# colmap/pycolmap

Hardware: AMD Instinct MI355X
Metric: descriptor-pair distances/sec (exhaustive SIFT match: dot + top-2 + ratio + cross-check) (higher is better)
Workload: dtype u8 descriptors, int8 MFMA / int32 accumulate; 1 GPU; 500 images x 4096 descriptors, exhaustive match + ratio test + cross-check (BASELINE.json configs[1] at N=1); pairs_total=124750, pairs_per_rank=124750, kernel=auto, matches_rank0=1865611

## Files before the change

pycolmap_amd/csrc/amc_internal.h:

```cpp
#pragma once

#include <hip/hip_runtime.h>
#include <stdint.h>

#include <algorithm>
#include <cstdlib>
#include <type_traits>
#include <vector>

#include "../../include/amc.h"
#include "guided_region.h"

namespace amc {

constexpr int kDim = AMC_DESC_DIM;
constexpr int kRowPad = 256;
constexpr int kAcosLutSize = 262145;

__host__ __device__ __forceinline__ constexpr uint32_t arena_swizzle(uint32_t row) {
    return ((row >> 1) & 1u) | (((row >> 4) & 3u) << 1);
}

struct ImageDev {
    const uint8_t* raw;
    const uint8_t* prep;
    const int32_t* rs128;
    const float* kp;
    uint32_t rows;
    uint32_t rows_pad;
    uint32_t kp_rows;
    uint32_t pad_;
};

enum : int { kGuidedNone = 0, kGuidedF = 1, kGuidedH = 2 };
struct GuidedDev {
    int32_t kind;
    float max_residual;
    float m[9];
    int32_t grid_ok;
    double bound[2];
    double minv[9];
};

using guided::kGridDim;
struct GridDev {
    const float* sxy;
    const uint32_t* sidx;
    const uint32_t* cell_start;
    float x0, y0, inv_cw, inv_ch;
    float cw, ch;
    float bx1, by1;
    uint32_t n;
    uint32_t pad_;
};
using guided::grid_cell;
#if defined(__HIPCC__)
__device__ __forceinline__ bool guided_rejects(const GuidedDev& g, float x1, float y1, float x2, float y2) {
    const float* m = g.m;
    if (g.kind == kGuidedF) {
        const float Fx1_0 = m[0] * x1 + m[1] * y1 + m[2] * 1.0f;
        const float Fx1_1 = m[3] * x1 + m[4] * y1 + m[5] * 1.0f;
        const float Fx1_2 = m[6] * x1 + m[7] * y1 + m[8] * 1.0f;
        const float Ftx2_0 = m[0] * x2 + m[3] * y2 + m[6] * 1.0f;
        const float Ftx2_1 = m[1] * x2 + m[4] * y2 + m[7] * 1.0f;
        const float x2tFx1 = x2 * Fx1_0 + y2 * Fx1_1 + 1.0f * Fx1_2;
        return x2tFx1 * x2tFx1 / (Fx1_0 * Fx1_0 + Fx1_1 * Fx1_1 + Ftx2_0 * Ftx2_0 + Ftx2_1 * Ftx2_1) > g.max_residual;
    }
    const float Hp_0 = m[0] * x1 + m[1] * y1 + m[2] * 1.0f;
    const float Hp_1 = m[3] * x1 + m[4] * y1 + m[5] * 1.0f;
    const float Hp_2 = m[6] * x1 + m[7] * y1 + m[8] * 1.0f;
    const float e0 = Hp_0 / Hp_2 - x2;
    const float e1 = Hp_1 / Hp_2 - y2;
    return e0 * e0 + e1 * e1 > g.max_residual;
}
#endif

struct Top2 {
    uint32_t best_v;
    uint32_t best_idx;
    uint32_t second_v;
    uint32_t pad;
};

struct PairDev {
    uint32_t slot1, slot2;
    uint32_t mode;
    uint32_t pad;
    uint64_t row_off;
    uint64_t col_off;
};

struct Dot4Work {
    uint32_t pair;
    uint32_t dir;
    uint32_t rb;
};

struct FinalizeParams {
    float max_ratio;
    float max_distance;
    int cross_check;
    int reserved;
};

int api_fail(int code, const char* fmt, ...) __attribute__((format(printf, 2, 3)));

constexpr const char* hipchk_who = nullptr;
#define HIPCHK(expr)                                                                                                   \
    do {                                                                                                               \
        const hipError_t e_ = (expr);                                                                                  \
        if (e_ != hipSuccess)                                                                                          \
            return ::amc::api_fail(AMC_E_HIP, "%s%s%s:%d: %s -> %s", hipchk_who ? hipchk_who : "",                    \
                                   hipchk_who ? ": " : "", __FILE__, __LINE__, #expr, hipGetErrorString(e_));        \
    } while (0)

inline bool env_flag(const char* name) { return std::getenv(name) != nullptr; }
inline long long env_int(const char* name, long long dflt, long long lo, long long hi) {
    const char* e = std::getenv(name);
    return e ? std::min(hi, std::max(lo, std::atoll(e))) : dflt;
}

template <typename T, bool kPinned>
struct GrowBuf {
    T* p = nullptr;
    size_t cap = 0;

    GrowBuf() = default;
    GrowBuf(GrowBuf&& o) noexcept : p(o.p), cap(o.cap) {
        o.p = nullptr;
        o.cap = 0;
    }
    GrowBuf& operator=(GrowBuf&& o) noexcept {
        if (this != &o) {
            release();
            p = o.p;
            cap = o.cap;
            o.p = nullptr;
            o.cap = 0;
        }
        return *this;
    }
    ~GrowBuf() { release(); }

    hipError_t ensure(size_t n) {
        if (n <= cap) return hipSuccess;
        release();
        const size_t want = std::max(n, std::is_void<T>::value ? (size_t)256 : (size_t)16);
        const size_t bytes = want * sizeof(typename std::conditional<std::is_void<T>::value, char, T>::type);
        void* q = nullptr;
        const hipError_t e = kPinned ? hipHostMalloc(&q, bytes, 0) : hipMalloc(&q, bytes);
        if (e == hipSuccess) {
            p = static_cast<T*>(q);
            cap = want;
        }
        return e;
    }
    void release() {
        if (p) (void)(kPinned ? hipHostFree(p) : hipFree(p));
        p = nullptr;
        cap = 0;
    }
};
template <typename T>
using DevBuf = GrowBuf<T, false>;
template <typename T>
using PinBuf = GrowBuf<T, true>;

inline size_t align256(size_t x) { return (x + 255) & ~(size_t)255; }

class DevParts {
  public:
    template <typename T>
    DevParts& part(T** ptr, size_t n) {
        parts_.push_back({ptr, align256(n * sizeof(T)), [](void* q, char* at) { *static_cast<T**>(q) = reinterpret_cast<T*>(at); }});
        return *this;
    }
    hipError_t carve(DevBuf<void>& buf) const {
        size_t total = 0;
        for (const Part& q : parts_) total += q.bytes;
        const hipError_t e = buf.ensure(total);
        if (e != hipSuccess) return e;
        char* at = static_cast<char*>(buf.p);
        for (const Part& q : parts_) {
            q.set(q.ptr, at);
            at += q.bytes;
        }
        return hipSuccess;
    }

  private:
    struct Part {
        void* ptr;
        size_t bytes;
        void (*set)(void* ptr, char* at);
    };
    std::vector<Part> parts_;
};

inline hipError_t create_events(hipEvent_t* ev, int n, const unsigned* flags = nullptr) {
    for (int i = 0; i < n; ++i) {
        const hipError_t e = hipEventCreateWithFlags(&ev[i], flags ? flags[i] : hipEventDefault);
        if (e != hipSuccess) {
            for (int j = 0; j < i; ++j) (void)hipEventDestroy(ev[j]);
            std::fill(ev, ev + n, nullptr);
            return e;
        }
    }
    return hipSuccess;
}

class StreamTimer {
  public:
    explicit StreamTimer(hipStream_t s) : s_(s), made_(create_events(ab_, 2)) {}
    StreamTimer(const StreamTimer&) = delete;
    StreamTimer& operator=(const StreamTimer&) = delete;
    ~StreamTimer() {
        for (hipEvent_t e : ab_)
            if (e) (void)hipEventDestroy(e);
        for (hipEvent_t e : spans_) (void)hipEventDestroy(e);
    }

    hipError_t start() { return made_ != hipSuccess ? made_ : hipEventRecord(ab_[0], s_); }
    hipError_t stop(double& ms) {
        hipError_t e = hipEventRecord(ab_[1], s_);
        if (e == hipSuccess) e = hipEventSynchronize(ab_[1]);
        return e == hipSuccess ? add_elapsed(ab_[0], ab_[1], ms) : e;
    }
    hipError_t span_begin() {
        hipEvent_t two[2];
        if (const hipError_t e = create_events(two, 2)) return e;
        spans_.insert(spans_.end(), two, two + 2);
        return hipEventRecord(two[0], s_);
    }
    hipError_t span_end() { return hipEventRecord(spans_.back(), s_); }
    hipError_t spans(double& ms) const {
        for (size_t i = 0; i + 1 < spans_.size(); i += 2)
            if (const hipError_t e = add_elapsed(spans_[i], spans_[i + 1], ms)) return e;
        return hipSuccess;
    }

  private:
    static hipError_t add_elapsed(hipEvent_t a, hipEvent_t b, double& ms) {
        float f = 0.f;
        const hipError_t e = hipEventElapsedTime(&f, a, b);
        if (e == hipSuccess) ms += f;
        return e;
    }
    hipStream_t s_;
    hipEvent_t ab_[2] = {nullptr, nullptr};
    hipError_t made_;
    std::vector<hipEvent_t> spans_;
};

struct Batches {
    std::vector<size_t> start{0};
    uint64_t most_items = 0, most_elems = 0;
    size_t count() const { return start.size() - 1; }
};
inline Batches split_batches(const uint64_t* offsets, size_t n, uint64_t max_items, uint64_t max_elems,
                             uint64_t factor = 1) {
    Batches b;
    for (size_t i = 0; i < n;) {
        size_t j = i + 1;
        while (j < n && j - i < max_items && (offsets[j + 1] - offsets[i]) * factor <= max_elems) ++j;
        b.most_items = std::max<uint64_t>(b.most_items, j - i);
        b.most_elems = std::max<uint64_t>(b.most_elems, offsets[j] - offsets[i]);
        b.start.push_back(j);
        i = j;
    }
    return b;
}

struct CtxView {
    int device;
    hipStream_t stream;
    const uint32_t* resident;
    uint64_t resident_rows;
};
CtxView ctx_view(amc_ctx* c);
struct TvgPair;
struct VerifyResident {
    size_t npairs = 0;
    uint64_t total = 0;
    const amc_tvg* tvg = nullptr;
    const uint8_t* mask = nullptr;
    const uint64_t* moff = nullptr;
    const TvgPair* tp = nullptr;
    const uint32_t* matches = nullptr;
};
VerifyResident verify_resident(amc_ctx* c);

hipError_t memset_async(void* p, int value, size_t bytes, hipStream_t s);
hipError_t memcpy_async(void* dst, const void* src, size_t bytes, hipMemcpyKind kind, hipStream_t s);

hipError_t launch_prep(const uint8_t* raw, uint8_t* prep, int32_t* rs128, uint32_t rows_pad,
                 uint32_t* maxsq_out, hipStream_t s);

hipError_t launch_match_dot4(const ImageDev* imgs, const PairDev* pairs, const Dot4Work* work,
                       uint32_t nwork, Top2* rowbuf, Top2* colbuf, const GuidedDev* guided, hipStream_t s);
hipError_t launch_match_guided_grid(const ImageDev* imgs, const GridDev* grids, const PairDev* pairs, const Dot4Work* work,
                              uint32_t nwork, Top2* rowbuf, Top2* colbuf, const GuidedDev* guided, hipStream_t s);

constexpr int kSegRows = 128;
constexpr int kSegsPerItem = 8;
struct alignas(64) SegDesc {
    const uint8_t* xprep;
    const int32_t* xrs;
    Top2* out;
    const uint32_t* list;
    const uint8_t* yprep;
    const int32_t* yrs;
    uint32_t cnt;
    uint32_t accword;
    uint32_t yrows;
    uint32_t pad_;
};
__device__ __forceinline__ bool one_way_accepts(const Top2 t, const float* __restrict__ lut,
                                                float max_ratio, float max_distance) {
    if (t.best_v == 0u) return false;
    const float a_best = lut[min(t.best_v, 262144u)];
    if (a_best > max_distance) return false;
    const float a_second = lut[min(t.second_v, 262144u)];
    if (a_best >= max_ratio * a_second) return false;
    return true;
}

hipError_t launch_build_segments(int mode, const ImageDev* imgs, const PairDev* pairs, const uint32_t* order,
                           const uint32_t* grp_start, uint32_t ngroups, const uint32_t* cand_cnt,
                           const uint32_t* candbuf, Top2* outbuf, uint32_t* seg_base, uint32_t* grp_segs,
                           uint32_t* grp_item_base, SegDesc* segs, uint32_t* nitems_dev, hipStream_t s);
struct ScanAccept;
struct CopyJob {
    const void* src = nullptr;
    void* dst = nullptr;
    unsigned long long n16 = 0;
    uint32_t parts = 0, pad_ = 0;
};
hipError_t launch_match_mfma(int mode, const SegDesc* segs, const uint32_t* nitems_dev, uint32_t max_items,
                       uint32_t* queue_head, uint32_t* accmask, const ScanAccept* accept_dev, hipStream_t s,
                       const CopyJob& job = CopyJob(), uint32_t* copy_head = nullptr);

hipError_t launch_resolve_index(int side, const ImageDev* imgs, const PairDev* pairs, uint32_t npairs,
                          Top2* table, uint32_t* accmask, const float* acos_lut, FinalizeParams fp,
                          const uint32_t* cand_cnt, const uint32_t* candbuf, uint32_t* err_count,
                          bool grouped, const uint32_t* order, uint32_t norder, hipStream_t s);
uint32_t resolve_grouped_max_rows();
constexpr uint32_t kSelectMaxCols = 1u << 20;

hipError_t launch_select_candidates(const ImageDev* imgs, const PairDev* pairs, uint32_t npairs, uint32_t max_cols,
                              const Top2* rowbuf, const uint32_t* accmask, const float* acos_lut,
                              FinalizeParams fp, uint32_t* cand_cnt, uint32_t* candbuf, hipStream_t s);

hipError_t launch_finalize(const ImageDev* imgs, const PairDev* pairs, uint32_t npairs,
                     const Top2* rowbuf, const Top2* colbuf, uint32_t* accmask,
                     const float* acos_lut, FinalizeParams fp, uint32_t* cursor, uint32_t capacity,
                     uint32_t* pair_off, uint32_t* pair_cnt, uint32_t* matches, hipStream_t s);

hipError_t launch_host_copy(void* dst_pinned, const void* src_dev, size_t bytes, hipStream_t s);
hipError_t launch_reorder_matches(const uint32_t* src_off, const uint32_t* cnt, const uint64_t* dst_off, uint32_t npairs,
                            const uint32_t* src, uint32_t* dst, hipStream_t s);

struct CameraDev {
    int32_t model_id;
    int32_t has_prior;
    uint64_t width, height;
    double params[12];
};
struct TvgImage {
    const float* kp;
    const double* kp64;
    const double* kpn;
    uint32_t rows;
    uint32_t pad;
    CameraDev cam;
};
hipError_t launch_undistort(const float* kp, const double* kp64, uint32_t rows, const CameraDev& cam, double* kpn,
                            hipStream_t s);
hipError_t launch_project(const double* uv, uint32_t n, const CameraDev& cam, double* xy, hipStream_t s);
struct TvgPair {
    uint32_t slot1, slot2;
    uint64_t match_off;
    uint64_t mask_off;
    uint32_t M;
    uint32_t tab_off[3];
    uint32_t orig;
};
struct PosePair {
    uint32_t slot1, slot2;
    uint64_t match_off;
    uint64_t mask_off;
    uint64_t ws_off;
    uint32_t M;
    int32_t config;
    double E[9], H[9];
};
struct alignas(128) PoseOut {
    int32_t ok;
    int32_t t_is_zero;
    uint32_t num_points3D;
    uint32_t pad;
    double R[9], t[3], q[4], cmed[2];
};
hipError_t launch_pose(const TvgImage* imgs, const PosePair* pairs, uint32_t npairs, const uint32_t* matches,
                       const uint8_t* mask, double* cosine_ws, PoseOut* out, hipStream_t s);

struct alignas(128) TvgOut {
    amc_tvg g;
    unsigned long long prof[8];
    unsigned long long work[12];
};
struct TvgParams {
    int32_t min_num_inliers, detect_watermark, force_H_use, min_num_trials;
    int32_t max_trials[4];
    double min_E_F_inlier_ratio, max_H_inlier_ratio, watermark_min_inlier_ratio,
        watermark_border_size, max_error;
    int32_t force_slow_sampler;
    int32_t no_fast_count;
    int32_t no_fast32;
    int32_t mode;
    uint32_t* bad_index_count;
    const double* wm_cut;
    const uint32_t* stream;
    uint32_t stream_len;
    uint32_t* stream_err;
};
struct alignas(64) TvgEState {
    double model[9];
    double sum;
    int32_t cnt, success, num_trials;
    uint32_t soff;
};
void tvg_diag_report();
void tvg_diag_report_e();
size_t tvg_ws_doubles_host(uint32_t mcap);
size_t tvg_ws_doubles_e_host(uint32_t mcap);
size_t tvg_ws_mask_bytes_host(uint32_t mcap);
constexpr int kTvgEWavesPerSimd = 2;
constexpr int kTvgFhWavesPerSimd = 4;
size_t tvg_lds_bytes(uint32_t mcap, int waves);
size_t tvg_lds_bytes_e(uint32_t mcap, int waves);
hipError_t launch_pack_verify(const TvgOut* out, const TvgPair* tp, uint32_t npairs, const uint8_t* mask_src,
                              const uint64_t* moff, amc_tvg* tvg_dst, uint8_t* mask_dst, unsigned long long* work,
                              int32_t trivial_below, hipStream_t s);
hipError_t launch_homography_decomposition(const double* in27, const double* p1, const double* p2, uint32_t n, double* out16,
                                           double* points3D, hipStream_t s);
hipError_t launch_sampson(const double* p1, const double* p2, size_t n, const double* E9, double* out,
                          hipStream_t s);
hipError_t launch_tvg_e(const TvgImage* imgs, const TvgPair* pairs, uint32_t npairs, const uint32_t* matches,
                        const uint32_t* trial_tabs, const TvgParams& P, double* ws, uint32_t mcap, uint32_t num_waves,
                        int waves_per_block, uint32_t* queue_head, TvgEState* estate, uint8_t* emask, TvgOut* out,
                        uint8_t* out_mask, hipStream_t s);
hipError_t launch_tvg_fh(const TvgImage* imgs, const TvgPair* pairs, uint32_t npairs, const uint32_t* matches,
                         const uint32_t* trial_tabs, const TvgParams& P, double* ws, uint8_t* mask_ws, uint32_t mcap,
                         uint32_t num_waves, int waves_per_block, uint32_t* queue_head, const TvgEState* estate,
                         const uint8_t* emask, TvgOut* out, uint8_t* out_mask, hipStream_t s);

size_t tvg_big_lds_bytes(int waves);
size_t tvg_big_lds_bytes_e(int waves);
size_t tvg_big_idx_doubles_host(uint32_t mcap);
hipError_t launch_tvg_e_big(const TvgImage* imgs, const TvgPair* pairs, uint32_t npairs, const uint32_t* matches,
                            const uint32_t* trial_tabs, const TvgParams& P, double* ws, uint32_t mcap, uint32_t num_waves,
                            int waves_per_block, uint32_t* queue_head, TvgEState* estate, uint8_t* emask, TvgOut* out,
                            uint8_t* out_mask, hipStream_t s);
hipError_t launch_tvg_fh_big(const TvgImage* imgs, const TvgPair* pairs, uint32_t npairs, const uint32_t* matches,
                             const uint32_t* trial_tabs, const TvgParams& P, double* ws, uint8_t* mask_ws, uint32_t mcap,
                             uint32_t num_waves, int waves_per_block, uint32_t* queue_head, const TvgEState* estate,
                             const uint8_t* emask, TvgOut* out, uint8_t* out_mask, hipStream_t s);

}
```

pycolmap_amd/csrc/match_mfma.hip:

```cpp
#include <cstdlib>

#include "amc_internal.h"
#include "scan_accept.h"

namespace amc {

typedef int i32x4 __attribute__((ext_vector_type(4)));
typedef __attribute__((address_space(1))) const void gvoid_t;
typedef __attribute__((address_space(3))) void lvoid_t;

constexpr int kBN = 256;
constexpr int kYS = kBN / 32;
constexpr int kUR = 64;
constexpr int kUPC = kBN / kUR;
constexpr int kChunkBytes = kBN * kDim;
constexpr int kW = kSegsPerItem;
constexpr int kXT = kSegRows / 16;
constexpr int kKeyShift = 7, kKeyCarried = 127;

constexpr int kNB = 3;
constexpr int kOffRs = 0;
constexpr int kOffQ = kOffRs + kNB * kBN * 4;
constexpr int kOffB = kOffQ + 16;
constexpr int kLdsBytes = kOffB + kNB * kChunkBytes;
static_assert(kBN == kRowPad, "a chunk is the row padding unit");
static_assert(kRowPad % kSegRows == 0 && kSegRows % 32 == 0, "segments tile the padded rows");
static_assert(kLdsBytes <= 160 * 1024, "LDS of one CU");
static_assert(sizeof(SegDesc) == 64, "a descriptor is 16 dwords: one per lane of a quarter wave");

enum : int { kDXprep = 0, kDXrs = 2, kDOut = 4, kDList = 6, kDYprep = 8, kDYrs = 10, kDCnt = 12, kDAccword = 13,
             kDYrows = 14 };

__device__ __forceinline__ void mfma_first(i32x4& d, const i32x4& a, const i32x4& b, const i32x4& c) {
    asm volatile("v_mfma_i32_16x16x64_i8 %0, %1, %2, %3" : "=&v"(d) : "v"(a), "v"(b), "v"(c));
}
__device__ __forceinline__ void mfma_acc(i32x4& d, const i32x4& a, const i32x4& b) {
    asm volatile("v_mfma_i32_16x16x64_i8 %0, %1, %2, %0" : "+v"(d) : "v"(a), "v"(b));
}

struct YFrag {
    i32x4 f[2][2];
    i32x4 ci[2];
};

__device__ __noinline__ __attribute__((used)) void copy_part(const uint4* __restrict__ src, uint4* __restrict__ dst,
                                                             unsigned long long b, unsigned long long e, int tid,
                                                             int nthreads) {
    __builtin_assume(tid >= 0 && tid < 1024 && nthreads >= 256 && nthreads <= 512);
    unsigned long long i = b + (unsigned long long)tid;
    const unsigned long long st = (unsigned long long)nthreads;
    for (; i + 3 * st < e; i += 4 * st) {
        const uint4 v0 = src[i], v1 = src[i + st], v2 = src[i + 2 * st], v3 = src[i + 3 * st];
        dst[i] = v0; dst[i + st] = v1; dst[i + 2 * st] = v2; dst[i + 3 * st] = v3;
    }
    for (; i < e; i += st) dst[i] = src[i];
}

template <int MODE>
__global__ __launch_bounds__(64 * kW) void match_mfma_kernel(const SegDesc* __restrict__ segs,
                                                             const uint32_t* __restrict__ nitems_p,
                                                             uint32_t* __restrict__ queue_head,
                                                             uint32_t* __restrict__ accmask,
                                                             const ScanAccept* __restrict__ accept,
                                                             CopyJob job, uint32_t* __restrict__ copy_head) {
    static_assert((kChunkBytes / 1024) % kW == 0 && kYS % (kChunkBytes / 1024 / kW) == 0, "a chunk splits into 1 KiB DMA pieces per wave, dealt evenly over its steps");
    __shared__ __attribute__((aligned(16))) char smem[kLdsBytes];

    const int tid = threadIdx.x;
    const int lane = tid & 63;
    const int wid = __builtin_amdgcn_readfirstlane(tid >> 6);
    const int l15 = lane & 15, lq = lane >> 4;
    volatile uint32_t* s_q = reinterpret_cast<volatile uint32_t*>(smem + kOffQ);
    if constexpr (MODE == 0) {
        if (job.parts) {
            __shared__ uint32_t s_part;
            if (tid == 0) s_part = atomicAdd(copy_head, 1u);
            __syncthreads();
            const uint32_t part = s_part;
            if (part < job.parts)
                copy_part(static_cast<const uint4*>(job.src), static_cast<uint4*>(job.dst), job.n16 * part / job.parts,
                          job.n16 * (part + 1) / job.parts, tid, 64 * kW);
        }
    }
    const uint32_t nitems = *nitems_p;
    const ScanAccept sa = *accept;

    auto load_desc = [&](uint32_t q) -> int {
        int v = 0;
        if (q < nitems && lane < 16) v = reinterpret_cast<const int*>(segs + (size_t)q * kSegsPerItem + wid)[lane];
        return v;
    };
    auto dword = [&](int dv, int f) -> int { return __builtin_amdgcn_readlane(dv, f); };
    auto dptr = [&](int dv, int f) -> const char* {
        const uint64_t lo = (uint32_t)__builtin_amdgcn_readlane(dv, f);
        const uint64_t hi = (uint32_t)__builtin_amdgcn_readlane(dv, f + 1);
        return reinterpret_cast<const char*>(lo | (hi << 32));
    };

    constexpr int kPW = kChunkBytes / 1024 / kW;
    auto stage_piece = [&](const char* yprep, int c, int buf, int ps) __attribute__((always_inline)) {
        const int piece = ps * kW + wid;
        __builtin_amdgcn_global_load_lds((gvoid_t*)(yprep + (size_t)c * kChunkBytes + piece * 1024 + lane * 16),
                                         (lvoid_t*)(smem + kOffB + buf * kChunkBytes + piece * 1024), 16, 0, 0);
    };
    auto stage_rs = [&](const char* yrs, int c, int buf) __attribute__((always_inline)) {
        if (wid == 0)
            __builtin_amdgcn_global_load_lds((gvoid_t*)(yrs + (size_t)c * kBN * 4 + lane * 16),
                                             (lvoid_t*)(smem + kOffRs + buf * kBN * 4), 16, 0, 0);
    };
    auto stage = [&](const char* yprep, const char* yrs, int c, int buf) __attribute__((always_inline)) {
#pragma unroll
        for (int ps = 0; ps < kPW; ++ps) stage_piece(yprep, c, buf, ps);
        stage_rs(yrs, c, buf);
    };

    const int yrow_lane = (kUR / 4) * (l15 >> 2) + (l15 & 3);
    const int ysw_lane = arena_swizzle(yrow_lane);
    const int yoff0 = kOffB + yrow_lane * kDim + ((lq ^ ysw_lane) * 16);
    const int yoff1 = kOffB + yrow_lane * kDim + (((4 + lq) ^ ysw_lane) * 16);
    const int coff = kOffRs + (kUR / 4) * lq * 4;
    auto load_y_part = [&](YFrag& y, int buf, int ys, int part) __attribute__((always_inline)) {
        const int ub = (ys / 2) * kUR, sp = ys % 2;
        if (part < 2) {
            const int so = buf * kBN * 4 + (ub + 8 * sp) * 4;
            y.ci[part] = *reinterpret_cast<const i32x4*>(smem + (coff + so) + 16 * part);
        } else {
            const int tt = (part - 2) >> 1, s = (part - 2) & 1;
            const int so = buf * kChunkBytes + (ub + 8 * sp) * kDim;
            y.f[tt][s] = *reinterpret_cast<const i32x4*>(smem + ((s ? yoff1 : yoff0) + so) + tt * 4 * kDim);
        }
    };
    auto load_y = [&](YFrag& y, int buf, int ys) __attribute__((always_inline)) {
#pragma unroll
        for (int part = 0; part < 6; ++part) load_y_part(y, buf, ys, part);
    };

    i32x4 xf[kXT][2];
    int best[kXT], sec[kXT], btile[kXT], xterm[kXT], part[kXT];
    auto load_x = [&](int dv) __attribute__((always_inline)) {
        const int cnt = dword(dv, kDCnt);
        const char* xprep = dptr(dv, kDXprep);
        const int* xrs = reinterpret_cast<const int*>(dptr(dv, kDXrs));
#pragma unroll
        for (int xt = 0; xt < kXT; ++xt) {
            const int kl = xt * 16 + l15;
            int row;
            if (MODE == 0) {
                row = kl;
            } else {
                const uint32_t* list = reinterpret_cast<const uint32_t*>(dptr(dv, kDList));
                row = cnt > 0 ? (int)list[min(kl, cnt - 1)] : 0;
            }
            const char* rp = xprep + (size_t)row * kDim;
            const int sw = arena_swizzle(row);
#pragma unroll
            for (int s = 0; s < 2; ++s) xf[xt][s] = *reinterpret_cast<const i32x4*>(rp + (((4 * s + lq) ^ sw) * 16));
            xterm[xt] = xrs[row] - (1 << 21);
            best[xt] = ((-xterm[xt]) << kKeyShift) | kKeyCarried;
            sec[xt] = best[xt];
            btile[xt] = -1;
        }
    };

    if (tid == 0) *s_q = atomicAdd(queue_head, 1u);
    __syncthreads();
    uint32_t q = *s_q;
    int dv = load_desc(q);
    if (q < nitems) {
        stage(dptr(dv, kDYprep), dptr(dv, kDYrs), 0, 0);
        if (dword(dv, kDYrows) > kBN) stage(dptr(dv, kDYprep), dptr(dv, kDYrs), 1, 1);
        if (dword(dv, kDCnt) > 0) load_x(dv);
    }
    __syncthreads();

    while (q < nitems) {
        const char* yprep = dptr(dv, kDYprep);
        const char* yrs = dptr(dv, kDYrs);
        const int yrows_item = dword(dv, kDYrows);
        const int nchunks = (yrows_item + kBN - 1) / kBN;
        const int last_steps = (((yrows_item - (nchunks - 1) * kBN) + 31) / 32 + 1) & ~1;
        const bool active = dword(dv, kDCnt) > 0;
        if (tid == 0) *s_q = atomicAdd(queue_head, 1u);

        i32x4 acc[2][2];
        auto insert = [&](int xt, int code) __attribute__((always_inline)) {
            asm volatile(
                "v_lshl_or_b32 %2, %2, 7, %3\n\t"
                "v_med3_i32 %1, %0, %1, %2\n\t"
                "v_max_i32 %0, %0, %2"
                : "+v"(best[xt]), "+v"(sec[xt]), "+v"(part[xt])
                : "s"(code));
        };
        auto flush = [&](int sb) __attribute__((always_inline)) {
#pragma unroll
            for (int xt = 0; xt < kXT; ++xt) {
                const int c = best[xt] & 127;
                btile[xt] = c != kKeyCarried ? sb * 64 + (126 - c) : btile[xt];
                best[xt] |= kKeyCarried;
            }
        };
        auto phase = [&](i32x4 (&an)[2], const YFrag& y, int xtn, const i32x4 (&ac)[2], int xtc, int sp, int gb)
                         __attribute__((always_inline)) {
            mfma_first(an[0], y.f[0][0], xf[xtn][0], y.ci[0]);
            mfma_first(an[1], y.f[1][0], xf[xtn][0], y.ci[1]);
            __builtin_amdgcn_sched_barrier(0);
            if (xtc == 0 ? sp == 0 : sp == 1) {
                insert((xtc + kXT - 1) % kXT, 126 - ((xtc == 0 ? gb - 1 : gb) & 63));
                if (xtc == 0 && gb != 0 && (gb & 63) == 0) flush((gb >> 6) - 1);
                __builtin_amdgcn_sched_barrier(0);
            }
            mfma_acc(an[0], y.f[0][1], xf[xtn][1]);
            mfma_acc(an[1], y.f[1][1], xf[xtn][1]);
            __builtin_amdgcn_sched_barrier(0);
            int t0, t1;
            if (sp == 0)
                asm volatile(
                    "v_max3_i32 %0, %3, %4, %5\n\t"
                    "v_max3_i32 %1, %6, %7, %8\n\t"
                    "v_max3_i32 %0, %0, %9, %10\n\t"
                    "v_max_i32 %2, %0, %1"
                    : "=&v"(t0), "=&v"(t1), "=&v"(part[xtc])
                    : "v"(ac[0][0]), "v"(ac[0][1]), "v"(ac[0][2]), "v"(ac[0][3]), "v"(ac[1][0]), "v"(ac[1][1]),
                      "v"(ac[1][2]), "v"(ac[1][3]));
            else
                asm volatile(
                    "v_max3_i32 %0, %3, %4, %5\n\t"
                    "v_max3_i32 %1, %6, %7, %8\n\t"
                    "v_max3_i32 %0, %0, %9, %10\n\t"
                    "v_max3_i32 %2, %0, %1, %2"
                    : "=&v"(t0), "=&v"(t1), "+v"(part[xtc])
                    : "v"(ac[0][0]), "v"(ac[0][1]), "v"(ac[0][2]), "v"(ac[0][3]), "v"(ac[1][0]), "v"(ac[1][1]),
                      "v"(ac[1][2]), "v"(ac[1][3]));
            __builtin_amdgcn_sched_barrier(0);
        };

        YFrag y0, y1;
        asm volatile("s_waitcnt vmcnt(0)" ::: "memory");
        __syncthreads();
        const uint32_t qn = *s_q;
        const int dvn = load_desc(qn);
        if (active) {
            load_y(y0, 0, 0);
            mfma_first(acc[0][0], y0.f[0][0], xf[0][0], y0.ci[0]);
            mfma_first(acc[0][1], y0.f[1][0], xf[0][0], y0.ci[1]);
            mfma_acc(acc[0][0], y0.f[0][1], xf[0][1]);
            mfma_acc(acc[0][1], y0.f[1][1], xf[0][1]);
            part[kXT - 1] = -(1 << 24);
            __builtin_amdgcn_sched_barrier(0);
        }
        auto step = [&](YFrag& yc, YFrag& yn, int c, int cb, int nb, int ys, int sp) __attribute__((always_inline)) {
            const bool lastt = (ys == kYS - 1);
            const bool cross = lastt && (c + 1 < nchunks);
            const bool fetch = c + 2 < nchunks;
            if (fetch) {
                const int fb = cb == 0 ? 2 : cb - 1;
                constexpr int kEvery = kYS / kPW;
                static_assert(kEvery == 2, "a DMA piece per block, behind its first step");
                if (sp == 0) stage_piece(yprep, c + 2, fb, ys / kEvery);
                if (ys == 0) stage_rs(yrs, c + 2, fb);
            }
            if (cross) {
                if (!fetch) asm volatile("s_waitcnt vmcnt(0)" ::: "memory");
                else if (wid == 0) asm volatile("s_waitcnt vmcnt(%0)" ::"n"(kPW + 1) : "memory");
                else asm volatile("s_waitcnt vmcnt(%0)" ::"n"(kPW) : "memory");
                asm volatile("s_barrier" ::: "memory");
            }
            if (active) {
                const int nbuf = cross ? nb : cb;
                const int nys = lastt ? (cross ? 0 : ys) : ys + 1;
                const int gb = c * kUPC + ys / 2;
#pragma unroll
                for (int xt = 0; xt < kXT; ++xt) {
                    if (xt + 1 < kXT)
                        phase(acc[(xt + 1) & 1], yc, xt + 1, acc[xt & 1], xt, sp, gb);
                    else
                        phase(acc[0], yn, 0, acc[xt & 1], xt, sp, gb);
                    if (xt < 6) {
                        load_y_part(yn, nbuf, nys, xt);
                        __builtin_amdgcn_sched_barrier(0);
                    }
                }
            }
        };
        for (int c = 0, cb = 0; c < nchunks; ++c) {
            const int nb = cb == 2 ? 0 : cb + 1;
            const int yend = (c == nchunks - 1) ? last_steps : kYS;
#pragma unroll 1
            for (int ys = 0; ys < yend; ys += 2) {
                step(y0, y1, c, cb, nb, ys, 0);
                step(y1, y0, c, cb, nb, ys + 1, 1);
            }
            cb = nb;
        }
        if (active) {
            const int lastb = (nchunks - 1) * kUPC + last_steps / 2 - 1;
            insert(kXT - 1, 126 - (lastb & 63));
            flush(lastb >> 6);
#pragma unroll
            for (int xt = 0; xt < kXT; ++xt) {
                best[xt] >>= kKeyShift;
                sec[xt] >>= kKeyShift;
            }
        }
        __syncthreads();

        int eb[kXT], es[kXT], et[kXT], ex[kXT];
#pragma unroll
        for (int xt = 0; xt < kXT; ++xt) {
            asm volatile("v_mov_b32 %0, %1" : "=v"(eb[xt]) : "v"(best[xt]));
            asm volatile("v_mov_b32 %0, %1" : "=v"(es[xt]) : "v"(sec[xt]));
            asm volatile("v_mov_b32 %0, %1" : "=v"(et[xt]) : "v"(btile[xt]));
            ex[xt] = xterm[xt];
        }
        if (qn < nitems) {
            stage(dptr(dvn, kDYprep), dptr(dvn, kDYrs), 0, 0);
            if (dword(dvn, kDYrows) > kBN) stage(dptr(dvn, kDYprep), dptr(dvn, kDYrs), 1, 1);
            if (dword(dvn, kDCnt) > 0) load_x(dvn);
        }
        if (active) {
            const int cnt = dword(dv, kDCnt);
            uint32_t bits_lo = 0;
#pragma unroll
            for (int xt = 0; xt < kXT; ++xt) {
                const int kl = xt * 16 + l15;
                int b = eb[xt], s = es[xt], t = et[xt] < 0 ? -1 : et[xt] * 2 + (lq >> 1);
#pragma unroll
                for (int m = 16; m <= 32; m <<= 1) {
                    const int ob = __shfl_xor(b, m);
                    const int os = __shfl_xor(s, m);
                    const int ot = __shfl_xor(t, m);
                    const bool ow = (ob > b) || (ob == b && (unsigned)ot < (unsigned)t);
                    s = max(max(s, os), ow ? b : ob);
                    t = ow ? ot : t;
                    b = ow ? ob : b;
                }
                bool acc_bit = false;
                if (lq == 0 && kl < cnt) {
                    Top2* out = reinterpret_cast<Top2*>(const_cast<char*>(dptr(dv, kDOut)));
                    int row = kl;
                    if (MODE == 1) row = (int)reinterpret_cast<const uint32_t*>(dptr(dv, kDList))[kl];
                    Top2 o;
                    o.best_v = (uint32_t)(b + ex[xt]);
                    o.best_idx = o.best_v ? (uint32_t)t : 0xFFFFFFFFu;
                    o.second_v = (uint32_t)(s + ex[xt]);
                    o.pad = 0;
                    out[row] = o;
                    if (MODE == 0) acc_bit = scan_may_accept(sa, o.best_v, o.second_v);
                }
                if (MODE == 0) {
                    const uint32_t bits = (uint32_t)__ballot(acc_bit);
                    if (xt & 1) {
                        if (lane == 0) accmask[(uint32_t)dword(dv, kDAccword) + (xt >> 1)] = bits_lo | (bits << 16);
                    } else {
                        bits_lo = bits;
                    }
                }
            }
        }
        q = qn;
        dv = dvn;
    }
}

__device__ __forceinline__ uint32_t pair_segments(int mode, const ImageDev* imgs, const PairDev& p, uint32_t pi,
                                                  const uint32_t* cand_cnt, uint32_t* nrows_out) {
    const uint32_t nx = mode == 0 ? imgs[p.slot1].rows : cand_cnt[pi];
    const uint32_t ny = imgs[mode == 0 ? p.slot2 : p.slot1].rows;
    *nrows_out = nx;
    return ny ? (nx + kSegRows - 1) / kSegRows : 0u;
}

__global__ __launch_bounds__(256) void seg_count_kernel(int mode, const ImageDev* __restrict__ imgs,
                                                        const PairDev* __restrict__ pairs,
                                                        const uint32_t* __restrict__ order,
                                                        const uint32_t* __restrict__ grp_start,
                                                        const uint32_t* __restrict__ cand_cnt,
                                                        uint32_t* __restrict__ seg_base, uint32_t* __restrict__ grp_segs) {
    __shared__ uint32_t wsum[4];
    const uint32_t g = blockIdx.x, tid = threadIdx.x, lane = tid & 63, wid = tid >> 6;
    const uint32_t i0 = grp_start[g], i1 = grp_start[g + 1];
    uint32_t running = 0;
    for (uint32_t base = i0; base < i1; base += 256) {
        const uint32_t i = base + tid;
        uint32_t s = 0, nr;
        if (i < i1) {
            const uint32_t pi = order[i];
            s = pair_segments(mode, imgs, pairs[pi], pi, cand_cnt, &nr);
        }
        uint32_t inc = s;
#pragma unroll
        for (int m = 1; m < 64; m <<= 1) {
            const uint32_t o = __shfl_up(inc, m);
            if (lane >= (uint32_t)m) inc += o;
        }
        if (lane == 63) wsum[wid] = inc;
        __syncthreads();
        uint32_t wbase = 0, total = 0;
        for (uint32_t k = 0; k < 4; ++k) {
            if (k < wid) wbase += wsum[k];
            total += wsum[k];
        }
        if (i < i1) seg_base[i] = running + wbase + inc - s;
        running += total;
        __syncthreads();
    }
    if (tid == 0) grp_segs[g] = running;
}

__global__ __launch_bounds__(1024) void seg_scan_kernel(const uint32_t* __restrict__ grp_segs, uint32_t ngroups,
                                                        uint32_t* __restrict__ grp_item_base,
                                                        uint32_t* __restrict__ nitems_out) {
    __shared__ uint32_t wsum[16];
    const uint32_t tid = threadIdx.x, lane = tid & 63, wid = tid >> 6;
    uint32_t running = 0;
    for (uint32_t base = 0; base < ngroups; base += 1024) {
        const uint32_t g = base + tid;
        const uint32_t s = g < ngroups ? (grp_segs[g] + kSegsPerItem - 1) / kSegsPerItem : 0u;
        uint32_t inc = s;
#pragma unroll
        for (int m = 1; m < 64; m <<= 1) {
            const uint32_t o = __shfl_up(inc, m);
            if (lane >= (uint32_t)m) inc += o;
        }
        if (lane == 63) wsum[wid] = inc;
        __syncthreads();
        uint32_t wbase = 0, total = 0;
        for (uint32_t k = 0; k < 16; ++k) {
            if (k < wid) wbase += wsum[k];
            total += wsum[k];
        }
        if (g < ngroups) grp_item_base[g] = running + wbase + inc - s;
        running += total;
        __syncthreads();
    }
    if (tid == 0) *nitems_out = running;
}

constexpr uint32_t kFillY = 8;
__global__ __launch_bounds__(256) void seg_fill_kernel(int mode, const ImageDev* __restrict__ imgs,
                                                       const PairDev* __restrict__ pairs,
                                                       const uint32_t* __restrict__ order,
                                                       const uint32_t* __restrict__ grp_start,
                                                       const uint32_t* __restrict__ cand_cnt,
                                                       const uint32_t* __restrict__ candbuf,
                                                       const uint32_t* __restrict__ seg_base,
                                                       const uint32_t* __restrict__ grp_segs,
                                                       const uint32_t* __restrict__ grp_item_base,
                                                       Top2* __restrict__ outbuf, SegDesc* __restrict__ segs) {
    const uint32_t g = blockIdx.x, tid = threadIdx.x, lane = tid & 63, wid = blockIdx.y * 4 + (tid >> 6);
    const uint32_t i0 = grp_start[g], i1 = grp_start[g + 1];
    if (i0 >= i1) return;
    const uint32_t total = grp_segs[g];
    if (total == 0) return;
    SegDesc* gs = segs + (size_t)grp_item_base[g] * kSegsPerItem;
    const PairDev p0 = pairs[order[i0]];
    const ImageDev Y = imgs[mode == 0 ? p0.slot2 : p0.slot1];
    for (uint32_t i = i0 + wid; i < i1; i += 4 * kFillY) {
        const uint32_t pi = order[i];
        const PairDev p = pairs[pi];
        uint32_t nx;
        const uint32_t ns = pair_segments(mode, imgs, p, pi, cand_cnt, &nx);
        const ImageDev X = imgs[mode == 0 ? p.slot1 : p.slot2];
        const uint32_t sb = seg_base[i];
        for (uint32_t k = lane; k < ns; k += 64) {
            const uint32_t row0 = k * kSegRows;
            SegDesc d;
            d.yprep = Y.prep;
            d.yrs = Y.rs128;
            d.yrows = Y.rows;
            d.cnt = min(nx - row0, (uint32_t)kSegRows);
            d.pad_ = 0;
            if (mode == 0) {
                d.xprep = X.prep + (size_t)row0 * kDim;
                d.xrs = X.rs128 + row0;
                d.out = outbuf + p.row_off + row0;
                d.list = nullptr;
                d.accword = (uint32_t)((p.row_off + row0) >> 5);
            } else {
                d.xprep = X.prep;
                d.xrs = X.rs128;
                d.out = outbuf + p.col_off;
                d.list = candbuf + p.col_off + row0;
                d.accword = 0;
            }
            gs[sb + k] = d;
        }
    }
    const uint32_t padded = (total + kSegsPerItem - 1) / kSegsPerItem * kSegsPerItem;
    if (blockIdx.y == 0 && tid < padded - total) {
        SegDesc d;
        d.xprep = Y.prep;
        d.xrs = Y.rs128;
        d.out = nullptr;
        d.list = nullptr;
        d.yprep = Y.prep;
        d.yrs = Y.rs128;
        d.cnt = 0;
        d.accword = 0;
        d.yrows = Y.rows;
        d.pad_ = 0;
        gs[total + tid] = d;
    }
}

hipError_t launch_build_segments(int mode, const ImageDev* imgs, const PairDev* pairs, const uint32_t* order,
                                 const uint32_t* grp_start, uint32_t ngroups, const uint32_t* cand_cnt,
                                 const uint32_t* candbuf, Top2* outbuf, uint32_t* seg_base, uint32_t* grp_segs,
                                 uint32_t* grp_item_base, SegDesc* segs, uint32_t* nitems_dev, hipStream_t s) {
    if (ngroups == 0) return memset_async(nitems_dev, 0, sizeof(uint32_t), s);
    hipLaunchKernelGGL(seg_count_kernel, dim3(ngroups), dim3(256), 0, s, mode, imgs, pairs, order, grp_start,
                       cand_cnt, seg_base, grp_segs);
    hipLaunchKernelGGL(seg_scan_kernel, dim3(1), dim3(1024), 0, s, grp_segs, ngroups, grp_item_base, nitems_dev);
    hipLaunchKernelGGL(seg_fill_kernel, dim3(ngroups, kFillY), dim3(256), 0, s, mode, imgs, pairs, order, grp_start,
                       cand_cnt, candbuf, seg_base, grp_segs, grp_item_base, outbuf, segs);
    return hipGetLastError();
}

hipError_t launch_match_mfma(int mode, const SegDesc* segs, const uint32_t* nitems_dev, uint32_t max_items,
                             uint32_t* queue_head, uint32_t* accmask, const ScanAccept* accept_dev, hipStream_t s,
                             const CopyJob& job_in, uint32_t* copy_head) {
    if (max_items == 0) return hipSuccess;
    CopyJob job = (mode == 0 && copy_head) ? job_in : CopyJob();
    hipError_t e = job.parts ? memset_async(copy_head, 0, sizeof(uint32_t), s) : hipSuccess;
    if (e != hipSuccess) return e;
    int dev = 0, cus = 256;
    if ((e = hipGetDevice(&dev)) != hipSuccess) return e;
    if ((e = hipDeviceGetAttribute(&cus, hipDeviceAttributeMultiprocessorCount, dev)) != hipSuccess) return e;
    static const int grid_cap = [] {
        const char* e = std::getenv("AMC_SCAN_GRID");
        return e ? std::atoi(e) : 0;
    }();
    if (grid_cap > 0 && grid_cap < cus) cus = grid_cap;
    const uint32_t grid = max_items < (uint32_t)cus ? max_items : (uint32_t)cus;
    if (job.parts > grid) job.parts = grid;
    if ((e = memset_async(queue_head, 0, sizeof(uint32_t), s)) != hipSuccess) return e;
    if (mode == 0)
        hipLaunchKernelGGL((match_mfma_kernel<0>), dim3(grid), dim3(64 * kW), 0, s, segs, nitems_dev, queue_head,
                           accmask, accept_dev, job, copy_head);
    else
        hipLaunchKernelGGL((match_mfma_kernel<1>), dim3(grid), dim3(64 * kW), 0, s, segs, nitems_dev, queue_head,
                           accmask, accept_dev, job, copy_head);
    return hipGetLastError();
}

}
```

Measured before the change: 12780 billion distances/s.

## Widen the MFMA scan unit to 128 rows with four steps per loop block

Doubles the row block (kUR 64→128) so each lane quarter covers a 32-row tile. The Y scan loop is unrolled to four steps per block, with the tile index math, last-step rounding and DMA piece cadence adjusted to match. The arena swizzle is shifted to row bits 5-6 so the LDS bank spread fits the new row mapping. The aim is to halve top-2 insert/flush overhead per row and to cut loop and branch cost, at the price of more unrolled code and register pressure. Optional timestamp instrumentation behind AMC_SCAN_STAMPS and an A/B summary script are added.

```diff
diff --git a/profiles/scan128/recipes/ab_summary.py b/profiles/scan128/recipes/ab_summary.py
--- /dev/null
+++ b/profiles/scan128/recipes/ab_summary.py
@@ -0,0 +1,57 @@
+import json, sys, os, statistics
+d, out = sys.argv[1], sys.argv[2]
+def last_json(p):
+    if not os.path.exists(p): return None
+    for line in reversed(open(p).read().strip().split("\n")):
+        line = line.strip()
+        if line.startswith("{"):
+            try: return json.loads(line)
+            except Exception: pass
+    return None
+def leg_ms(j, leg):
+    if leg in ("headline", "headline_of_the_full_runs"): return j.get("ms_per_step")
+    if leg == "scan_ms_per_launch": return (j.get("roofline") or {}).get("avg_kernel_ms")
+    v = j.get(leg)
+    if not isinstance(v, dict): return None
+    for k in ("ms_per_step", "ms_per_call", "ms"):
+        if k in v: return v[k]
+    return None
+res = {
+    "cmd": ["python bench.py --gpus 1 --steps 20 --warmup 5", "python bench.py --full --no-db --no-config3 --no-config4"],
+    "how": "one GPU call (profiles/scan128/recipes/ab_parent.sh), alternating parent1 / new1 / parent2 / new2 / parent3 / new3; parent = the parent commit's library (tools/ab_prev_lib.sh) selected with AMC_LIB_PATH, new = the tree's own library; each step under its own timeout, chained with &&.  The db leg is left out: it goes through the host module, which links libamc.so directly and cannot be switched this way.",
+    "rule": "headline: the new median must be below the parent's median by more than three times the parent's max - min of this call (gain_over_three_spreads).  Every other leg: the new median may exceed the parent's median by at most the parent's max - min (within_parent_spread).",
+    "ms_per_step": {}, "summary": {}, "other": {}}
+runs = {}
+for kind in ("head", "full"):
+    for who in ("parent", "new"):
+        for i in (1, 2, 3):
+            runs[(kind, who, i)] = last_json(f"{d}/{kind}_{who}{i}.json")
+legs = [("headline", "head"), ("scan_ms_per_launch", "head")]
+legs += [(l, "full") for l in ("headline_of_the_full_runs", "verify", "pipeline", "dense", "ragged", "sift_stats")]
+for leg, kind in legs:
+    vals = {}
+    for who in ("parent", "new"):
+        for i in (1, 2, 3):
+            j = runs[(kind, who, i)]
+            if j is not None:
+                v = leg_ms(j, leg)
+                if v is not None: vals[f"{who}{i}"] = round(float(v), 3)
+    res["ms_per_step"][leg] = vals
+    p = [vals[k] for k in vals if k.startswith("parent")]
+    n = [vals[k] for k in vals if k.startswith("new")]
+    if len(p) == 3 and len(n) == 3:
+        pm, nm, sp = statistics.median(p), statistics.median(n), max(p) - min(p)
+        res["summary"][leg] = {"parent_median": pm, "new_median": nm, "parent_spread": round(sp, 3),
+                               "new_minus_parent": round(nm - pm, 3), "within_parent_spread": nm - pm <= sp,
+                               "gain_over_three_spreads": pm - nm > 3 * sp}
+for (kind, who, i), j in runs.items():
+    if j is None or kind != "full": continue
+    o = {}
+    for leg in ("ragged", "sift_stats", "dense", "pipeline", "verify", "cpu_baseline"):
+        v = j.get(leg)
+        if isinstance(v, dict):
+            o[leg] = {k: v[k] for k in ("vs_uniform", "gpu_vs_oracle_mismatching_pairs", "value") if k in v}
+    res["other"][f"{who}{i}"] = o
+json.dump(res, open(out, "w"), indent=1)
+print(json.dumps(res["summary"], indent=1))
+print(json.dumps(res["other"]))
diff --git a/pycolmap_amd/csrc/amc_internal.h b/pycolmap_amd/csrc/amc_internal.h
--- a/pycolmap_amd/csrc/amc_internal.h
+++ b/pycolmap_amd/csrc/amc_internal.h
@@ -18,7 +18,7 @@
 constexpr int kAcosLutSize = 262145;
 
 __host__ __device__ __forceinline__ constexpr uint32_t arena_swizzle(uint32_t row) {
-    return ((row >> 1) & 1u) | (((row >> 4) & 3u) << 1);
+    return ((row >> 1) & 1u) | (((row >> 5) & 3u) << 1);
 }
 
 struct ImageDev {
diff --git a/pycolmap_amd/csrc/match_mfma.hip b/pycolmap_amd/csrc/match_mfma.hip
--- a/pycolmap_amd/csrc/match_mfma.hip
+++ b/pycolmap_amd/csrc/match_mfma.hip
@@ -11,7 +11,8 @@
 
 constexpr int kBN = 256;
 constexpr int kYS = kBN / 32;
-constexpr int kUR = 64;
+constexpr int kUR = 128;
+constexpr int kSPB = kUR / 32;
 constexpr int kUPC = kBN / kUR;
 constexpr int kChunkBytes = kBN * kDim;
 constexpr int kW = kSegsPerItem;
@@ -24,6 +25,7 @@
 constexpr int kOffB = kOffQ + 16;
 constexpr int kLdsBytes = kOffB + kNB * kChunkBytes;
 static_assert(kBN == kRowPad, "a chunk is the row padding unit");
+static_assert(kUR == 128 && kSPB == 4, "a lane quarter's rows of a block are one 32-row tile; the loop body is one block");
 static_assert(kRowPad % kSegRows == 0 && kSegRows % 32 == 0, "segments tile the padded rows");
 static_assert(kLdsBytes <= 160 * 1024, "LDS of one CU");
 static_assert(sizeof(SegDesc) == 64, "a descriptor is 16 dwords: one per lane of a quarter wave");
@@ -42,6 +44,12 @@
     i32x4 f[2][2];
     i32x4 ci[2];
 };
+
+#ifdef AMC_SCAN_STAMPS
+constexpr int kStampMaxWG = 1024;
+__device__ uint32_t g_scan_stamps[2 * kStampMaxWG * kSegsPerItem * 8];
+#define AMC_STAMP() ((uint32_t)__builtin_amdgcn_s_memtime())
+#endif
 
 __device__ __noinline__ __attribute__((used)) void copy_part(const uint4* __restrict__ src, uint4* __restrict__ dst,
                                                              unsigned long long b, unsigned long long e, int tid,
@@ -120,7 +128,7 @@
     const int yoff1 = kOffB + yrow_lane * kDim + (((4 + lq) ^ ysw_lane) * 16);
     const int coff = kOffRs + (kUR / 4) * lq * 4;
     auto load_y_part = [&](YFrag& y, int buf, int ys, int part) __attribute__((always_inline)) {
-        const int ub = (ys / 2) * kUR, sp = ys % 2;
+        const int ub = (ys / kSPB) * kUR, sp = ys % kSPB;
         if (part < 2) {
             const int so = buf * kBN * 4 + (ub + 8 * sp) * 4;
             y.ci[part] = *reinterpret_cast<const i32x4*>(smem + (coff + so) + 16 * part);
@@ -162,6 +170,11 @@
         }
     };
 
+#ifdef AMC_SCAN_STAMPS
+    uint32_t st_a = 0, st_first = 0, st_end = 0, st_sum[5] = {0, 0, 0, 0, 0};
+    bool st_prev = false, st_prev_active = false;
+    uint32_t* const st_slot = g_scan_stamps + ((size_t)(MODE * kStampMaxWG + min((int)blockIdx.x, kStampMaxWG - 1)) * kW + wid) * 8;
+#endif
     if (tid == 0) *s_q = atomicAdd(queue_head, 1u);
     __syncthreads();
     uint32_t q = *s_q;
@@ -178,7 +191,7 @@
         const char* yrs = dptr(dv, kDYrs);
         const int yrows_item = dword(dv, kDYrows);
         const int nchunks = (yrows_item + kBN - 1) / kBN;
-        const int last_steps = (((yrows_item - (nchunks - 1) * kBN) + 31) / 32 + 1) & ~1;
+        const int last_steps = (((yrows_item - (nchunks - 1) * kBN) + 31) / 32 + kSPB - 1) & ~(kSPB - 1);
         const bool active = dword(dv, kDCnt) > 0;
         if (tid == 0) *s_q = atomicAdd(queue_head, 1u);
 
@@ -204,7 +217,7 @@
             mfma_first(an[0], y.f[0][0], xf[xtn][0], y.ci[0]);
             mfma_first(an[1], y.f[1][0], xf[xtn][0], y.ci[1]);
             __builtin_amdgcn_sched_barrier(0);
-            if (xtc == 0 ? sp == 0 : sp == 1) {
+            if (xtc == 0 ? sp == 0 : sp == kSPB - 1) {
                 insert((xtc + kXT - 1) % kXT, 126 - ((xtc == 0 ? gb - 1 : gb) & 63));
                 if (xtc == 0 && gb != 0 && (gb & 63) == 0) flush((gb >> 6) - 1);
                 __builtin_amdgcn_sched_barrier(0);
@@ -239,6 +252,24 @@
         __syncthreads();
         const uint32_t qn = *s_q;
         const int dvn = load_desc(qn);
+#ifdef AMC_SCAN_STAMPS
+        {
+            const uint32_t now = AMC_STAMP();
+            if (st_prev) {
+                st_sum[0] += st_a;
+                st_sum[1] += now - st_end;
+                st_sum[2] += now - st_first;
+                st_sum[3] += 1;
+                st_sum[4] += st_prev_active ? 1 : 0;
+                if (lane == 0) {
+#pragma unroll
+                    for (int k = 0; k < 5; ++k) st_slot[k] = st_sum[k];
+                }
+            }
+            st_a = 0;
+            st_first = now;
+        }
+#endif
         if (active) {
             load_y(y0, 0, 0);
             mfma_first(acc[0][0], y0.f[0][0], xf[0][0], y0.ci[0]);
@@ -249,26 +280,32 @@
             __builtin_amdgcn_sched_barrier(0);
         }
         auto step = [&](YFrag& yc, YFrag& yn, int c, int cb, int nb, int ys, int sp) __attribute__((always_inline)) {
-            const bool lastt = (ys == kYS - 1);
+            const bool lastt = sp == kSPB - 1 && ys == kYS - 1;
             const bool cross = lastt && (c + 1 < nchunks);
             const bool fetch = c + 2 < nchunks;
             if (fetch) {
                 const int fb = cb == 0 ? 2 : cb - 1;
                 constexpr int kEvery = kYS / kPW;
-                static_assert(kEvery == 2, "a DMA piece per block, behind its first step");
-                if (sp == 0) stage_piece(yprep, c + 2, fb, ys / kEvery);
+                static_assert(kEvery == 2, "a DMA piece behind every other step");
+                if (sp % kEvery == 0) stage_piece(yprep, c + 2, fb, ys / kEvery);
                 if (ys == 0) stage_rs(yrs, c + 2, fb);
             }
             if (cross) {
+#ifdef AMC_SCAN_STAMPS
+                const uint32_t st_t = AMC_STAMP();
+#endif
                 if (!fetch) asm volatile("s_waitcnt vmcnt(0)" ::: "memory");
                 else if (wid == 0) asm volatile("s_waitcnt vmcnt(%0)" ::"n"(kPW + 1) : "memory");
                 else asm volatile("s_waitcnt vmcnt(%0)" ::"n"(kPW) : "memory");
                 asm volatile("s_barrier" ::: "memory");
+#ifdef AMC_SCAN_STAMPS
+                st_a += AMC_STAMP() - st_t;
+#endif
             }
             if (active) {
                 const int nbuf = cross ? nb : cb;
                 const int nys = lastt ? (cross ? 0 : ys) : ys + 1;
-                const int gb = c * kUPC + ys / 2;
+                const int gb = c * kUPC + ys / kSPB;
 #pragma unroll
                 for (int xt = 0; xt < kXT; ++xt) {
                     if (xt + 1 < kXT)
@@ -286,14 +323,16 @@
             const int nb = cb == 2 ? 0 : cb + 1;
             const int yend = (c == nchunks - 1) ? last_steps : kYS;
 #pragma unroll 1
-            for (int ys = 0; ys < yend; ys += 2) {
+            for (int ys = 0; ys < yend; ys += kSPB) {
                 step(y0, y1, c, cb, nb, ys, 0);
                 step(y1, y0, c, cb, nb, ys + 1, 1);
+                step(y0, y1, c, cb, nb, ys + 2, 2);
+                step(y1, y0, c, cb, nb, ys + 3, 3);
             }
             cb = nb;
         }
         if (active) {
-            const int lastb = (nchunks - 1) * kUPC + last_steps / 2 - 1;
+            const int lastb = (nchunks - 1) * kUPC + last_steps / kSPB - 1;
             insert(kXT - 1, 126 - (lastb & 63));
             flush(lastb >> 6);
 #pragma unroll
@@ -303,6 +342,11 @@
             }
         }
         __syncthreads();
+#ifdef AMC_SCAN_STAMPS
+        st_end = AMC_STAMP();
+        st_prev = true;
+        st_prev_active = active;
+#endif
 
         int eb[kXT], es[kXT], et[kXT], ex[kXT];
 #pragma unroll
@@ -323,7 +367,7 @@
 #pragma unroll
             for (int xt = 0; xt < kXT; ++xt) {
                 const int kl = xt * 16 + l15;
-                int b = eb[xt], s = es[xt], t = et[xt] < 0 ? -1 : et[xt] * 2 + (lq >> 1);
+                int b = eb[xt], s = es[xt], t = et[xt] < 0 ? -1 : et[xt] * kSPB + lq;
 #pragma unroll
                 for (int m = 16; m <= 32; m <<= 1) {
                     const int ob = __shfl_xor(b, m);
@@ -357,6 +401,13 @@
                 }
             }
         }
+#ifdef AMC_SCAN_STAMPS
+        if (qn >= nitems && lane == 0) {
+            st_slot[5] = st_a;
+            st_slot[6] = AMC_STAMP() - st_first;
+            st_slot[7] = 1;
+        }
+#endif
         q = qn;
         dv = dvn;
     }
```

After: 13220 billion distances/s (median of 6 runs). 3.4% higher.
